# ygjwd12345/UCD

Measured on AMD Instinct MI355X. Metric: images/sec (whole node) per UCD train step, VOC 15-5 step-1, 513^2 bs=24, higher is better.
Workload: dtype bf16

## Files before the change

### include/ucd_hip.h

```cpp
#ifndef UCD_HIP_H
#define UCD_HIP_H

#include <stddef.h>
#include <stdint.h>

#ifdef __cplusplus
extern "C" {
#endif

#define UCD_VERSION 100

typedef void* ucd_stream_t;
typedef void* ucd_comm_t;

enum ucd_dtype { UCD_F32 = 0, UCD_BF16 = 1 };
enum ucd_act { UCD_ACT_IDENTITY = 0, UCD_ACT_LEAKY_RELU = 1, UCD_ACT_ELU = 2  };
#define UCD_ACT_MASK 0xff
#define UCD_NORM_ABS_GAMMA 0x100
enum ucd_pixcon_precision { UCD_PIXCON_F32 = 0, UCD_PIXCON_F16 = 1, UCD_PIXCON_F16_SPLIT = 2 };
enum ucd_error {
  UCD_OK = 0,
  UCD_EINVAL = -1,
  UCD_EALIGN = -2,
  UCD_EWORKSPACE = -3,
// ... 345 lines not shown
enum ucd_conv_form {
  UCD_CONV_SINGLE = 0,
  UCD_CONV_DB = 1,
  UCD_CONV_LW128 = 2,
  UCD_CONV_LW256 = 3,
  UCD_CONV_LW64 = 4
};
#define UCD_CONV_FORM_NAMES {"single", "2x64", "lw/128", "lw/256", "lw/64"}
typedef struct ucd_conv1x1_plan_t {
  int form;
  int tile_rows, tile_cols;
  int tiles_m, tiles_n, grid, threads, lds_bytes;
  int param_off;
} ucd_conv1x1_plan_t;
int ucd_conv1x1_plan(const ucd_conv1x1_desc* desc, ucd_conv1x1_plan_t* plan);
int ucd_conv1x1_row_tiles(int M);
int ucd_conv1x1_stat_replicas(int M);
size_t ucd_conv1x1_stats_partial_bytes(int M, int C);
int ucd_conv1x1(const ucd_conv1x1_desc* desc, ucd_stream_t stream);

int ucd_conv3_tap_plan(int B, int H, int W, int dilation, int tile_rows, int* perm, int* masks, int* n_classes);
int ucd_conv3_tap_classes(int mode);
int ucd_conv3_tap_plans_resident(void);
int ucd_conv3_tap_stats(long long* launches, int* last_tile_rows, int* last_class_ordered);

int ucd_conv1x1_stats_finalize(const float* partial, int M, int C, const float* weight, float* running_mean,
                               float* running_var, float momentum, float eps, float* buf, float* pack, int flags,
                               ucd_stream_t stream);

int ucd_abn_reduce_partials(const float* partial, int tiles, int C, float* sums, float* sums_copy, const float* weight,
// ... 105 lines not shown
```

### ucd_amd/csrc/conv1x1.hip

```cpp
#include "common.h"
#include "abn_finalize.h"
#include "conv3_taps.h"
#include <algorithm>
#include <mutex>
#include <vector>

namespace ucd {
namespace {

typedef float f32x16 __attribute__((ext_vector_type(16)));
typedef __bf16 bf16x8 __attribute__((ext_vector_type(8)));
typedef __hip_bfloat16 bf16;

constexpr int kThreads = 256;
constexpr int kBM = 128;

constexpr int kBK = 64;
constexpr int kDbStages = 2;
constexpr int kLwStages = 3;

struct Args {
  const bf16* A; int lda;
  const bf16* W; int ldw;
  bf16* Y; int ldy;
  int M, N, K;
  const float *in_mean, *in_scale, *in_shift; int in_act; float in_slope;
  const float *out_mean, *out_scale, *out_shift, *out_invstd;
// ... 29 lines not shown


template <int OUT> constexpr int kEpilogueBarriers = 4 + (OUT >= 2 ? 2 : 0);
template <int OUT, int HALVES> constexpr int kEpilogueBarriersH = 2 * HALVES + (OUT >= 2 ? 2 : 0);

__device__ __forceinline__ void live_taps(int m0, int m1, int ohw, int oW, int iH, int dil, int& tap0, int& ntap) {
  tap0 = 0; ntap = 9;
  if (dil <= 1 || m1 - m0 >= ohw) return;
  const int first = m0 % ohw, last = (m1 - 1) % ohw;
  int ymin = first / oW, ymax = last / oW;
  if (first > last) { ymin = 0; ymax = iH - 1; }
  if (ymax < dil) { tap0 = 3; ntap -= 3; }
  if (ymin >= iH - dil) ntap -= 3;
}

template <int BN, bool PRO, int OUT, bool CONV3 = false, bool DB = false, bool RT = false>
__global__ __launch_bounds__(kThreads, DB ? 2 : ((PRO || OUT >= 3) && BN == 128 ? 3 : 4)) void conv1x1_kernel(Args p) {
  static_assert(!DB || !PRO, "the double-buffered form has no input transform");
  static_assert(!RT || (CONV3 && OUT == 0 && !PRO), "class-ordered rows: the plain 3x3 product");
  constexpr int kStage = (kBM + BN) * kBK * 2;
  constexpr int WN = BN / 2;
  constexpr int TN = WN / 32;
  extern __shared__ __attribute__((aligned(1024))) unsigned char smem[];
  unsigned char* As = smem;
  unsigned char* Bs = smem + kBM * kBK * 2;
  float* Ps = reinterpret_cast<float*>(smem + p.param_off);

  const int xcd = blockIdx.x & 7, j = blockIdx.x >> 3;
  const int tm = (j / p.tiles_n) * 8 + xcd, tn = j % p.tiles_n;
  if (tm >= p.tiles_m) return;
  const int m0 = tm * kBM, n0 = tn * BN;
  const int tid = threadIdx.x, lane = tid & 63, wave = __builtin_amdgcn_readfirstlane(tid >> 6);
  const int wm = wave >> 1, wn = wave & 1;

  f32x16 acc[2][TN];
#pragma unroll
  for (int a = 0; a < 2; ++a)
#pragma unroll
    for (int b = 0; b < TN; ++b)
#pragma unroll
      for (int r = 0; r < 16; ++r) acc[a][b][r] = 0.f;

  constexpr int RPC = 1024 / (kBK * 2), SPR = kBK / 8;
  constexpr int CA = kBM / RPC / 4, CB = BN / RPC / 4;
  const bf16* ga[CA];
  const bf16* gb[CB];
  int py[CA], px[CA], pimg[CA], pslot[CA];
#pragma unroll
  for (int i = 0; i < CA; ++i) {
    const int row = RPC * (wave * CA + i) + lane / SPR;
    const int slot = ((lane % SPR) ^ swz_fn(row)) << 3;
    ga[i] = p.A + (size_t)min(m0 + row, p.M - 1) * p.lda + slot;
    if (CONV3 || p.stride > 1) {
      const int m = m0 + row;
      const int mm = min(m, p.M - 1);
      const int pix = RT ? p.perm[mm] : mm;
// ... 12 lines not shown
    gb[i] = p.W + (size_t)(n0 + row) * p.ldw + (((lane % SPR) ^ swz_fn(row)) << 3);
  }
  const int ks = tid & 7, srow = tid >> 3;
  const bf16* arow[4];
#pragma unroll
  for (int i = 0; i < 4; ++i) arow[i] = p.A + (size_t)min(m0 + srow + 32 * i, p.M - 1) * p.lda + ks * 8;

  if (PRO) {
    for (int k = tid; k < p.K; k += kThreads) {
      Ps[k] = p.in_mean[k];
      Ps[p.K + k] = p.in_scale[k];
      Ps[2 * p.K + k] = p.in_shift ? p.in_shift[k] : 0.f;
    }
    __syncthreads();
  }
  const int fr = lane & 31, fh = lane >> 5;
  const int kpt = p.K / kBK;
  int tap0 = 0, ntap = 9;
  unsigned trem = 0;
  if constexpr (RT) { trem = (unsigned)p.masks[tm]; ntap = __builtin_popcount(trem); }
  else if (CONV3 && p.stride == 1) live_taps(m0, min(m0 + kBM, p.M), p.ohw, p.oW, p.iH, p.dil, tap0, ntap);
  const int nk = CONV3 ? ntap * kpt : kpt;
  int akt = -1, ctap = 0;
  auto tap_of = [&](int kt) {
    if constexpr (RT) {
      if (kt != akt) { ctap = __builtin_ctz(trem); trem &= trem - 1; akt = kt; }
      return ctap;
    } else {
      return tap0 + kt;
    }
  };
// ... 103 lines not shown
      } else {
#pragma unroll
        for (int i = 0; i < CA; ++i)
          __builtin_amdgcn_raw_ptr_buffer_load_lds(rsA1, (lptr_t)(As + (wave * CA + i) * 1024), 16, (int)a1off[i], k0 * 2, 0, 0);
      }
#pragma unroll
      for (int i = 0; i < CB; ++i)
        __builtin_amdgcn_raw_ptr_buffer_load_lds(rsW, (lptr_t)(Bs + (wave * CB + i) * 1024), 16, (int)boff[i], wk0 * 2, 0, 0);
    }
    if (!DB) {
      if (!PRO) asm volatile("s_waitcnt vmcnt(0)" ::: "memory");
      asm volatile("s_waitcnt lgkmcnt(0)" ::: "memory");
      __builtin_amdgcn_s_barrier();
    }
    if (DB) {
      bf16x8 af[2][2], bfr[2][TN];
      auto read_slice = [&](int set, int kk) {
#pragma unroll
        for (int a = 0; a < 2; ++a) af[set][a] = *reinterpret_cast<const bf16x8*>(Ac + swz(wm * 64 + a * 32 + fr, 2 * kk + fh));
#pragma unroll
        for (int b = 0; b < TN; ++b) bfr[set][b] = *reinterpret_cast<const bf16x8*>(Bc + swz(wn * WN + b * 32 + fr, 2 * kk + fh));
      };
      read_slice(0, 0);
#pragma unroll
      for (int kk = 0; kk < kBK / 16; ++kk) {
        if (kk + 1 < kBK / 16) read_slice((kk + 1) & 1, kk + 1);
        __builtin_amdgcn_sched_barrier(0);
#pragma unroll
        for (int a = 0; a < 2; ++a)
#pragma unroll
          for (int b = 0; b < TN; ++b)
            acc[a][b] = __builtin_amdgcn_mfma_f32_32x32x16_bf16(af[kk & 1][a], bfr[kk & 1][b], acc[a][b], 0, 0, 0);
        __builtin_amdgcn_sched_barrier(0);
      }
    } else {
#pragma unroll
      for (int kk = 0; kk < kBK / 16; ++kk) {
        bf16x8 af[2], bfr[TN];
#pragma unroll
        for (int a = 0; a < 2; ++a) af[a] = *reinterpret_cast<const bf16x8*>(Ac + swz(wm * 64 + a * 32 + fr, 2 * kk + fh));
#pragma unroll
        for (int b = 0; b < TN; ++b) bfr[b] = *reinterpret_cast<const bf16x8*>(Bc + swz(wn * WN + b * 32 + fr, 2 * kk + fh));
#pragma unroll
        for (int a = 0; a < 2; ++a)
#pragma unroll
          for (int b = 0; b < TN; ++b) acc[a][b] = __builtin_amdgcn_mfma_f32_32x32x16_bf16(af[a], bfr[b], acc[a][b], 0, 0, 0);
      }
    }
  }

#include "conv1x1_epilogue.inc"
}

template <int BM, int BN, int OUT, bool CONV3, bool RT = false>
__global__ __launch_bounds__(BM == 64 ? 384 : BM * 4, (BM + BN) * kBK * 2 * kLwStages > 80 * 1024 ? 1 : 2) void conv_lw_kernel(Args p) {
  static_assert(BM == 64 || BM == 128 || BM == 256, "64-, 128- or 256-row workgroup tiles");
  static_assert(BM != 64 || BN == 64, "the 64-row form runs its epilogue on 128 threads: 64-column tiles");
  static_assert(!RT || (CONV3 && OUT == 0), "class-ordered rows: the plain 3x3 product");
  constexpr int NC = BM / 32, NL = BM == 64 ? 4 : BM / 32;
  constexpr int kStage = (BM + BN) * kBK * 2;
  constexpr int WN = BN / 2, TN = WN / 32;
  extern __shared__ __attribute__((aligned(1024))) unsigned char smem[];
  unsigned char* As = smem;
  unsigned char* Bs = smem + BM * kBK * 2;
  const int xcd = blockIdx.x & 7, j = blockIdx.x >> 3;
  const int tmw = (j / p.tiles_n) * 8 + xcd, tn = j % p.tiles_n;
  if (tmw >= p.tiles_m) return;
  const int m0w = tmw * BM, n0 = tn * BN;
  const int tid = threadIdx.x, lane = tid & 63, wave = __builtin_amdgcn_readfirstlane(tid >> 6);
  const int kpt = p.K / kBK;
  int tap0 = 0, ntap = 9;
  unsigned trem = 0;
  if constexpr (RT) { trem = (unsigned)p.masks[tmw]; ntap = __builtin_popcount(trem); }
  else if (CONV3 && p.stride == 1) live_taps(m0w, min(m0w + BM, p.M), p.ohw, p.oW, p.iH, p.dil, tap0, ntap);
  const int nk = CONV3 ? ntap * kpt : kpt;

// ... 72 lines not shown
    int wst = kLwStages - 1;
    for (int kb = 0; kb < nk; ++kb) {
      const int r = min(kLwStages - 2, nk - 1 - kb);
      if (r == 1) asm volatile("s_waitcnt vmcnt(%0)" ::"n"(CA + CB) : "memory");
      else asm volatile("s_waitcnt vmcnt(0)" ::: "memory");
      __builtin_amdgcn_s_barrier();
      if (kb + kLwStages - 1 < nk) fill(kb + kLwStages - 1, wst);
      wst = wst + 1 == kLwStages ? 0 : wst + 1;
    }
#pragma unroll
    for (int b = 0; b < kEpilogueBarriersH<OUT, BM == 64 ? 1 : 2>; ++b) __syncthreads();
    return;
  }

  const int wmw = wave >> 1, wn = wave & 1;
  f32x16 acc[2][TN];
#pragma unroll
  for (int a = 0; a < 2; ++a)
#pragma unroll
    for (int b = 0; b < TN; ++b)
#pragma unroll
      for (int r = 0; r < 16; ++r) acc[a][b][r] = 0.f;
  const int fr = lane & 31, fh = lane >> 5;
  int rst = 0;
  for (int kb = 0; kb < nk; ++kb) {
    asm volatile("s_waitcnt lgkmcnt(0)" ::: "memory");
    __builtin_amdgcn_s_barrier();
    const unsigned char* Ac = As + rst * kStage;
    const unsigned char* Bc = Bs + rst * kStage;
    rst = rst + 1 == kLwStages ? 0 : rst + 1;
    bf16x8 af[2][2], bfr[2][TN];
    auto read_slice = [&](int set, int kk) {
#pragma unroll
      for (int a = 0; a < 2; ++a) af[set][a] = *reinterpret_cast<const bf16x8*>(Ac + swz(wmw * 64 + a * 32 + fr, 2 * kk + fh));
#pragma unroll
      for (int b = 0; b < TN; ++b) bfr[set][b] = *reinterpret_cast<const bf16x8*>(Bc + swz(wn * WN + b * 32 + fr, 2 * kk + fh));
    };
    read_slice(0, 0);
#pragma unroll
    for (int kk = 0; kk < kBK / 16; ++kk) {
      if (kk + 1 < kBK / 16) read_slice((kk + 1) & 1, kk + 1);
      __builtin_amdgcn_sched_barrier(0);
#pragma unroll
      for (int a = 0; a < 2; ++a)
#pragma unroll
        for (int b = 0; b < TN; ++b)
          acc[a][b] = __builtin_amdgcn_mfma_f32_32x32x16_bf16(af[kk & 1][a], bfr[kk & 1][b], acc[a][b], 0, 0, 0);
      __builtin_amdgcn_sched_barrier(0);
    }
  }
  if constexpr (BM == 64) {
    const int tm = tmw, m0 = m0w, wm = 0;
#define UCD_EPI_THREADS 128
#define UCD_EPI_HALVES 1
#include "conv1x1_epilogue.inc"
#undef UCD_EPI_THREADS
#undef UCD_EPI_HALVES
  } else {
    const int sub = wmw >> 1;
    const int tm = tmw * (BM / 128) + sub, m0 = m0w + sub * 128, wm = wmw & 1;
    constexpr size_t kOutBytes = ((size_t)64 * (BN + 4) * 4 + 1023) / 1024 * 1024;
    unsigned char* smem_all = smem;
    {
// ... 282 lines not shown
        if (co + j < Co) q[j] = tmp[j];
    }
  }
}

int pick_wgrad_chunks(int M, int N, int K) {
  const int tiles = (N / 128) * (K / 128);
  int chunks = (512 + tiles - 1) / tiles;
  const int max_chunks = (M + 255) / 256;
  if (chunks > max_chunks) chunks = max_chunks;
  if (chunks < 1) chunks = 1;
  return chunks;
}


struct Tuning { int pipe, bn64_below, lw64_below; };
const Tuning& tuning() {
  static const Tuning t = [] {
    const char *e = getenv("UCD_CONV_PIPE"), *bn = getenv("UCD_CONV_BN64_TILES"), *lw = getenv("UCD_CONV_LW64_TILES");
    const int pipe = !e || !*e || !strcmp(e, "auto") ? -1 : !strcmp(e, "2x64") ? UCD_CONV_DB : !strcmp(e, "lw64") ? UCD_CONV_LW128
                     : !strcmp(e, "lw256") ? UCD_CONV_LW256 : -2;
    return Tuning{pipe, bn ? atoi(bn) : 128, lw ? atoi(lw) : 128};
  }();
  return t;
}

constexpr struct { int rows, threads, stages; } kForms[] = {{128, 256, 1}, {128, 256, kDbStages}, {128, 512, kLwStages},
                                                            {256, 1024, kLwStages}, {64, 384, kLwStages}};

int plan_launch(const ucd_conv1x1_desc* d, ucd_conv1x1_plan_t* p, const char* fn) {
  const Tuning& t = tuning();
  UCD_REQUIRE(t.pipe != -2, UCD_EINVAL, "%s: UCD_CONV_PIPE=%s names no form (accepted: auto, 2x64, lw64, lw256)", fn,
              getenv("UCD_CONV_PIPE"));
  const bool conv3 = d->taps == 9, pro = d->in_scale != nullptr;
  const int out = d->out_mode;
  UCD_REQUIRE(d->M > 0 && d->N > 0 && d->K > 0 && (d->taps == 0 || d->taps == 1 || conv3) && out >= 0 && out <= 4, UCD_EINVAL,
              "%s: empty product, taps not 1 or 9, or unknown out_mode", fn);
// ... 20 lines not shown
                         (size_t)(kThreads / (BN / 8)) * 2 * BN * 4});
  p->param_off = 0;
  if (pro) {
    p->param_off = (int)align_up(lds, 16);
    lds = p->param_off + (size_t)3 * d->K * sizeof(float);
  }
  UCD_REQUIRE(form != UCD_CONV_SINGLE || lds <= 64 * 1024, UCD_EUNSUPPORTED, "%s: K = %d is too wide for the fused input transform", fn,
              d->K);
  p->form = form; p->tile_rows = rows; p->tile_cols = BN;
  p->tiles_m = ceil_div(d->M, rows); p->tiles_n = tiles_n;
  p->grid = ceil_div(p->tiles_m, 8) * 8 * tiles_n;
  p->threads = kForms[form].threads; p->lds_bytes = (int)lds;
  return 0;
}

template <int BN, int OUT, bool CONV3, bool RT = false, bool PRO = false>
int launch_form(const ucd_conv1x1_plan_t& p, hipStream_t s, const Args& a, const char* fn) {
  const int lds = p.lds_bytes;
  if (p.form == UCD_CONV_SINGLE) {
    conv1x1_kernel<BN, PRO, OUT, CONV3, false, RT><<<p.grid, p.threads, lds, s>>>(a);
    return 0;
  }
  if constexpr (!PRO) {
    switch (p.form) {
      case UCD_CONV_DB:
        conv1x1_kernel<BN, false, OUT, CONV3, true, RT><<<p.grid, p.threads, lds, s>>>(a);
        return 0;
      case UCD_CONV_LW128:
        UCD_TRY_LDS((conv_lw_kernel<128, BN, OUT, CONV3, RT>), lds);
        conv_lw_kernel<128, BN, OUT, CONV3, RT><<<p.grid, p.threads, lds, s>>>(a);
        return 0;
      case UCD_CONV_LW256:
        if constexpr (OUT <= 2 && BN == 128) {
          UCD_TRY_LDS((conv_lw_kernel<256, BN, OUT, CONV3, RT>), lds);
          conv_lw_kernel<256, BN, OUT, CONV3, RT><<<p.grid, p.threads, lds, s>>>(a);
          return 0;
        }
        break;
      case UCD_CONV_LW64:
        if constexpr (BN == 64) {
          conv_lw_kernel<64, BN, OUT, CONV3, RT><<<p.grid, p.threads, lds, s>>>(a);
          return 0;
        }
        break;
    }
  }
  static const char* const names[] = UCD_CONV_FORM_NAMES;
  set_error("%s: no %s kernel for %d-column tiles and out_mode %d", fn, names[p.form], BN, OUT);
  return UCD_EINVAL;
}

template <int BN>
int launch_plan(const ucd_conv1x1_plan_t& p, int out_mode, bool conv3, bool pro, hipStream_t s, const Args& a, const char* fn) {
  UCD_REQUIRE(!(conv3 && out_mode == 4), UCD_EINVAL, "%s: out_mode 4 belongs to the 1x1 products", fn);
  UCD_REQUIRE(!(pro && (conv3 || out_mode == 4)), UCD_EINVAL, "%s: no input transform on a 3x3 product or with out_mode 4", fn);
  if (conv3) switch (out_mode) {
    case 0: return a.perm ? launch_form<BN, 0, true, true>(p, s, a, fn) : launch_form<BN, 0, true>(p, s, a, fn);
    case 1: return launch_form<BN, 1, true>(p, s, a, fn);
    case 2: return launch_form<BN, 2, true>(p, s, a, fn);
    default: return launch_form<BN, 3, true>(p, s, a, fn);
  }
  if (pro) switch (out_mode) {
    case 0: return launch_form<BN, 0, false, false, true>(p, s, a, fn);
    case 1: return launch_form<BN, 1, false, false, true>(p, s, a, fn);
    case 2: return launch_form<BN, 2, false, false, true>(p, s, a, fn);
    default: return launch_form<BN, 3, false, false, true>(p, s, a, fn);
  }
  switch (out_mode) {
    case 0: return launch_form<BN, 0, false>(p, s, a, fn);
    case 1: return launch_form<BN, 1, false>(p, s, a, fn);
    case 2: return launch_form<BN, 2, false>(p, s, a, fn);
    case 3: return launch_form<BN, 3, false>(p, s, a, fn);
    default: return launch_form<BN, 4, false>(p, s, a, fn);
  }
}

int g_tap_classes = -1;
std::mutex g_tap_mutex;
int tap_classes_mode() {
  std::lock_guard<std::mutex> lock(g_tap_mutex);
  if (g_tap_classes < 0) {
    const char* e = getenv("UCD_CONV3_TAP_CLASSES");
    g_tap_classes = e && !strcmp(e, "0") ? 0 : e && !strcmp(e, "2") ? 2 : 1;
  }
  return g_tap_classes;
}

struct TapPlan { int dev, B, H, W, d, rows; int* perm; int* masks; int max_on, max_off; };
// ... 125 lines not shown
  if (conv3 && stride == 1 && d->dilation > 1 && d->out_mode == 0) {
    const int mode = tap_classes_mode(), rows = plan.tile_rows;
    const TapPlan* tp = mode ? tap_plan_get(d->M / (d->H * d->W), d->H, d->W, d->dilation, rows, s) : nullptr;
    if (tp && mode == 1 && rows == 64 && tp->max_on >= tp->max_off) {
      int dev = 0, cus = 0;
      if (hipGetDevice(&dev) == hipSuccess && hipDeviceGetAttribute(&cus, hipDeviceAttributeMultiprocessorCount, dev) == hipSuccess &&
          (long long)plan.tiles_m * plan.tiles_n <= cus)
        tp = nullptr;
    }
    if (tp) { a.perm = tp->perm; a.masks = tp->masks; }
    std::lock_guard<std::mutex> lock(g_tap_mutex);
    g_tap_launches += tp != nullptr;
    g_tap_last_rows = rows; g_tap_last_rt = tp != nullptr;
  }
  const bool pro = d->in_scale != nullptr;
  if (int rc = plan.tile_cols == 128 ? launch_plan<128>(plan, d->out_mode, conv3, pro, s, a, fn)
                                     : launch_plan<64>(plan, d->out_mode, conv3, pro, s, a, fn))
    return rc;
  return check_launch(fn);
}

int ucd_conv1x1_plan(const ucd_conv1x1_desc* d, ucd_conv1x1_plan_t* plan) {
  static const char* fn = "ucd_conv1x1_plan";
  UCD_REQUIRE(d && plan, UCD_EINVAL, "%s: NULL argument", fn);
  return plan_launch(d, plan, fn);
}

int ucd_conv3_tap_classes(int mode) {
  const int cur = tap_classes_mode();
  if (mode < 0) return cur;
  std::lock_guard<std::mutex> lock(g_tap_mutex);
  g_tap_classes = mode >= 2 ? 2 : mode;
  return g_tap_classes;
}

int ucd_conv3_tap_stats(long long* launches, int* last_tile_rows, int* last_class_ordered) {
  std::lock_guard<std::mutex> lock(g_tap_mutex);
  if (launches) *launches = g_tap_launches;
  if (last_tile_rows) *last_tile_rows = g_tap_last_rows;
  if (last_class_ordered) *last_class_ordered = g_tap_last_rt;
// ... 102 lines not shown
```

### ucd_amd/csrc/conv1x1_epilogue.inc

```
#ifndef UCD_EPI_ACTIVE
#define UCD_EPI_ACTIVE true
#define UCD_EPI_ACTIVE_DEFAULTED
#endif
#ifndef UCD_EPI_TILE_OK
#define UCD_EPI_TILE_OK true
#define UCD_EPI_TILE_OK_DEFAULTED
#endif
#ifndef UCD_EPI_ROW
#define UCD_EPI_ROW(r) (r)
#endif
#ifndef UCD_EPI_THREADS
#define UCD_EPI_THREADS kThreads
#define UCD_EPI_HALVES 2
#define UCD_EPI_THREADS_DEFAULTED
#endif
  constexpr int CP = BN + 4;
  float* Cs = reinterpret_cast<float*>(smem);
  constexpr int CPR = BN / 8;
  constexpr int RPT = 64 * CPR / (UCD_EPI_THREADS);
  constexpr int RSTEP = (UCD_EPI_THREADS) / CPR;
  const int c8 = tid % CPR, r0 = tid / CPR;
  const int ncol = n0 + c8 * 8;
  Pack8 em, es, eb, ei;
  if (OUT == 3) {
    em = load_f8(p.out_mean + ncol);
    es = load_f8(p.out_scale + ncol);
    eb = load_f8(p.out_shift + ncol);
    ei = load_f8(p.out_invstd + ncol);
  }
  float am[OUT == 1 ? TN : 1], as_[OUT == 1 ? TN : 1], ab[OUT == 1 ? TN : 1];
  if (OUT == 1) {
#pragma unroll
    for (int b = 0; b < TN; ++b) {
      const int col = n0 + wn * WN + b * 32 + (lane & 31);
      am[b] = p.out_mean[col];
      as_[b] = p.out_scale[col];
      ab[b] = p.out_shift[col];
    }
  }
  if (OUT == 4) {
    em = load_f8(p.out_mean + ncol);
    ei = load_f8(p.out_invstd + ncol);
  }
  Pack8 kshift, s1, s2;
#pragma unroll
  for (int j = 0; j < 4; ++j) { kshift.p[j] = f32x2{0.f, 0.f}; s1.p[j] = f32x2{0.f, 0.f}; s2.p[j] = f32x2{0.f, 0.f}; }
  const bool has_side = ((OUT == 0 || OUT == 4) && p.accumulate) || (OUT == 1 && p.R != nullptr) || OUT == 3;
  const bf16* sp = (OUT == 0 || OUT == 4) ? p.Y : p.R;
  const int lds_ = (OUT == 0 || OUT == 4) ? p.ldy : p.ldr;
// ... 4 lines not shown
#pragma unroll
      for (int i = 0; i < RPT; ++i)
        side[i] = *reinterpret_cast<const uint4*>(sp + (size_t)UCD_EPI_ROW(min(m0 + half * 64 + r0 + RSTEP * i, p.M - 1)) * lds_ + ncol);
    }
    if (OUT == 4) {
#pragma unroll
      for (int i = 0; i < RPT; ++i) {
        const size_t row = (size_t)min(m0 + half * 64 + r0 + RSTEP * i, p.M - 1);
        side_y[i] = *reinterpret_cast<const uint4*>(p.R + row * p.ldr + ncol);
        side_z[i] = *reinterpret_cast<const uint4*>(p.Z + row * p.ldz + ncol);
      }
    }
    __syncthreads();
    if (wm == half) {
#pragma unroll
      for (int a = 0; a < 2; ++a)
#pragma unroll
        for (int b = 0; b < TN; ++b)
#pragma unroll
          for (int r = 0; r < 16; ++r) {
            const int row = a * 32 + (r & 3) + 8 * (r >> 2) + 4 * (lane >> 5);
            Cs[row * CP + wn * WN + b * 32 + (lane & 31)] =
                OUT == 1 ? (acc[a][b][r] - am[OUT == 1 ? b : 0]) * as_[OUT == 1 ? b : 0] + ab[OUT == 1 ? b : 0] : acc[a][b][r];
          }
    }
    __syncthreads();
    if (OUT == 2 && half == 0 && p.stat_acc) {
      kshift = load_f8(p.stat_shift + ncol);
    } else if (OUT == 2 && half == 0) {
      const float4 k0 = *reinterpret_cast<const float4*>(Cs + c8 * 8), k1 = *reinterpret_cast<const float4*>(Cs + c8 * 8 + 4);
      Pack8 kf;
      kf.p[0] = f32x2{k0.x, k0.y}; kf.p[1] = f32x2{k0.z, k0.w}; kf.p[2] = f32x2{k1.x, k1.y}; kf.p[3] = f32x2{k1.z, k1.w};
      kshift = unpack8(pack8(kf));
    }
#pragma unroll
    for (int i = 0; i < RPT; ++i) {
      const int row = r0 + RSTEP * i;
// ... 96 lines not shown
        dst[(1 + which) * p.N] = t;
      } else {
        p.partial[(size_t)tm * 2 * p.N + which * p.N + n0 + col] = t;
      }
    }
    if (OUT == 2 && p.stat_acc) {
      if (tm == 0 && r0 == 0 && UCD_EPI_TILE_OK) {
#pragma unroll
        for (int j = 0; j < 4; ++j) *reinterpret_cast<f32x2*>(p.partial + ncol + 2 * j) = kshift.p[j];
      }
    } else if (OUT == 2 && r0 == 0 && UCD_EPI_TILE_OK) {
#pragma unroll
      for (int j = 0; j < 4; ++j) *reinterpret_cast<f32x2*>(p.partial + (size_t)tm * 3 * p.N + ncol + 2 * j) = kshift.p[j];
    }
  }
#ifdef UCD_EPI_ACTIVE_DEFAULTED
#undef UCD_EPI_ACTIVE
#undef UCD_EPI_ACTIVE_DEFAULTED
#endif
#ifdef UCD_EPI_TILE_OK_DEFAULTED
#undef UCD_EPI_TILE_OK
#undef UCD_EPI_TILE_OK_DEFAULTED
#endif
#ifdef UCD_EPI_THREADS_DEFAULTED
#undef UCD_EPI_THREADS
#undef UCD_EPI_HALVES
#undef UCD_EPI_THREADS_DEFAULTED
#endif
```

### ucd_amd/hip.py

```python
from __future__ import annotations

import ctypes as C
import os

import torch

_HERE = os.path.dirname(os.path.abspath(__file__))
LIB_PATH = os.path.join(_HERE, "libucd_hip.so")

F32, BF16 = 0, 1
ACT_IDENTITY, ACT_LEAKY_RELU, ACT_ELU = 0, 1, 2
ACT_CODES = {"identity": ACT_IDENTITY, "leaky_relu": ACT_LEAKY_RELU, "elu": ACT_ELU}
ACT_MASK = 0xFF
NORM_ABS_GAMMA = 0x100
PIX_TILE = 128
PIXCON_LD = 256
PIXCON_F32, PIXCON_F16, PIXCON_F16_SPLIT = 0, 1, 2
KD_UNBIASED, KD_PLAIN = 0, 1
EINVAL, EALIGN, EWORKSPACE = -1, -2, -3
EUNSUPPORTED = -4
SEG_FORMS = {1: "pk<16,8>", 2: "pk<20,4>", 3: "pk<12,12>", 4: "reg<24,16>", 5: "reg<24,24>", 6: "wide/fixed", 7: "wide/f32"}
PIXCON_PATHS = {1: "f32", 2: "f32/wide", 3: "f16/planned", 4: "f16/split"}
CONV_FORMS = ("single", "2x64", "lw/128", "lw/256", "lw/64")
WGRAD_FORMS = ("tile", "strided", "row3")
# ... 97 lines not shown
    "ucd_pod_plan": (_i, [_i, _i, _i, _p, _i, _i, _i, _p, _p, _p]),
    "ucd_pod_forward": (_i, [_p, _i, _p, _i, _i, _i, _i, _i, _i, _f, _p, _i, _f, _p, _p, _p, _z, _p]),
    "ucd_pod_backward": (_i, [_p, _i, _i, _i, _i, _i, _i, _f, _p, _i, _p, _p, _p, _i, _p]),
    "ucd_pod_logits_plan": (_i, [_i, _i, _i, _i, _p, _i, _i, _i, _p, _p, _p]),
    "ucd_pod_logits_forward": (_i, [_p, _i, _p, _i, _i, _i, _i, _i, _i, _i, _p, _i, _i, _f, _p, _p, _p, _z, _p]),
    "ucd_pod_logits_backward": (_i, [_p, _i, _i, _i, _i, _i, _i, _i, _p, _i, _p, _p, _p, _i, _p]),
    "ucd_proto_plan": (_i, [_q, _i, _i, _i, _p, _p, _p, _p]),
    "ucd_proto_classify": (_i, [_p, _i, _i, _i, _i, _i, _i, _i, _i, _p, _i, _p, _p]),
    "ucd_proto_forward": (_i, [_p, _i, _i, _p, _q, _i, _i, _i, _p, _p, _p, _p, _f, _f, _f, _p, _p, _p, _p, _p, _z, _p]),
    "ucd_proto_backward": (_i, [_p, _i, _i, _p, _q, _i, _i, _p, _p, _p, _i, _p]),
    "ucd_proto_update": (_i, [_p, _p, _p, _p, _i, _i, _p]),
    "ucd_conv1x1_row_tiles": (_i, [_i]),
    "ucd_conv1x1_stats_partial_bytes": (_z, [_i, _i]),
    "ucd_conv1x1": (_i, [C.POINTER(Conv1x1Desc), _p]),
    "ucd_conv1x1_plan": (_i, [C.POINTER(Conv1x1Desc), C.POINTER(Conv1x1Plan)]),
    "ucd_conv1x1_stats_finalize": (_i, [_p, _i, _i, _p, _p, _p, _f, _f, _p, _p, _i, _p]),
    "ucd_conv3_tap_plan": (_i, [_i, _i, _i, _i, _i, _p, _p, _p]),
    "ucd_conv3_tap_classes": (_i, [_i]),
    "ucd_conv3_tap_plans_resident": (_i, []),
    "ucd_conv3_tap_stats": (_i, [_p, _p, _p]),
    "ucd_abn_reduce_partials": (_i, [_p, _i, _i, _p, _p, _p, _i, _p]),
    "ucd_conv1x1_wgrad_workspace_bytes": (_z, [_i, _i, _i]),
    "ucd_conv1x1_wgrad": (_i, [_p, _i, _p, _i, _i, _i, _i, _p, _p, _p, _i, _f, _p, _p, _z, _p]),
    "ucd_abn_sync_finalize": (_i, [_p, _i, _i, _i, _p, _p, _p, _f, _f, _p, _i, _p]),
    "ucd_stem_pooled_size": (_i, [_i]),
    "ucd_stem_pool_workspace_bytes": (_z, [_i]),
    "ucd_stem_apply_pool": (_i, [_p, _i, _i, _i, _i, _p, _p, _p, _i, _f, _p, _p, _p]),
    "ucd_stem_pool_backward": (_i, [_p, _p, _p, _i, _i, _i, _i, _p, _p, _p, _p, _p, _p, _f, _i, _f, _p, _p, _z, _i, _p]),
    "ucd_conv_wgrad_workspace_bytes": (_z, [_i, _i, _i, _i]),
    "ucd_stem_conv7x7": (_i, [_p, C.c_longlong, C.c_longlong, C.c_longlong, C.c_longlong, _i, _i, _i, _p, _p, _p]),
# ... 557 lines not shown
def _conv1x1_plan(d):
    p = Conv1x1Plan()
    _check(load().ucd_conv1x1_plan(C.byref(d), C.byref(p)), "ucd_conv1x1_plan")
    out = {n: getattr(p, n) for n, _ in Conv1x1Plan._fields_}
    out["form"] = CONV_FORMS[p.form]
    return out


def conv1x1_plan(M, N, K, taps=1, out_mode=0, stride=1, in_transform=False, stat_acc=False):
    d = Conv1x1Desc()
    d.M, d.N, d.K, d.taps, d.out_mode, d.stride = int(M), int(N), int(K), int(taps), int(out_mode), int(stride)
    d.in_scale, d.stat_acc = (16 if in_transform else None), (16 if stat_acc else None)
    return _conv1x1_plan(d)


def conv1x1(a, w, y, in_norm=None, out_mode=0, out_norm=None, residual=None, partial=None, accumulate=False, conv3=None,
            side2=None, strided=None, stat_acc=None, stat_shift=None, stat_acc2=None, stat_rep=1):
    lib = load()
    d = Conv1x1Desc()
    M, K = y.shape[0], a.shape[1]
    N = w.shape[0]
    d.a, d.lda, d.w, d.ldw, d.y, d.ldy = a.data_ptr(), a.stride(0), w.data_ptr(), w.stride(0), y.data_ptr(), y.stride(0)
    d.M, d.N, d.K = M, N, K
    if conv3 is not None:
        d.taps, d.H, d.W, d.dilation = 9, int(conv3[0]), int(conv3[1]), int(conv3[2])
        if len(conv3) > 3:
            d.stride = int(conv3[3])
    elif strided is not None:
        d.H, d.W, d.stride = int(strided[0]), int(strided[1]), int(strided[2])
    if in_norm is not None:
# ... 277 lines not shown
```

### ucd_amd/switches.py

```python
from __future__ import annotations

import os

DEFAULTS = {
    "UCD_FUSED_CONV1X1": "1",
    "UCD_BWD_LINK": "1",
    "UCD_BLOCK_LINK": "1",
    "UCD_PROJ_ALIAS": "1",
    "UCD_DGRAD_VIA_FWD": "1",
    "UCD_OWN_STRIDED": "1",
    "UCD_OWN_WGRAD": "1",
    "UCD_F32_OWN_CONV": "0",
    "UCD_OWN_HEADS": "1",
    "UCD_OWN_STEM": "1",
    "UCD_WGRAD3": "1",
    "UCD_CONV_PIPE": "auto",
    "UCD_CONV_BN64_TILES": "128",
    "UCD_CONV_LW64_TILES": "128",
    "UCD_WGRAD_DEFER": "1",
    "UCD_WGRAD_STREAM": "1",
    "UCD_CONV3_TAP_CLASSES": "1",
    "UCD_STAT_ATOMIC": "1",
    "UCD_SEG_PK": "1",
    "UCD_SEG_KD_EX": "1",
    "UCD_FUSED_LDE": "1",
    "UCD_FUSED_POD": "1",
    "UCD_FUSED_PSEUDO": "1",
    "UCD_FUSED_FOCAL": "1",
    "UCD_FUSED_PROTO": "1",
    "UCD_VAL_DEVICE": "1",
    "UCD_STEM_EVAL_FUSED": "1",
# ... 42 lines not shown
```

Measured before the change: 849.0.

## Add 16x16x32 MFMA variant for dilated 3x3 conv kernels with auto selection

Templates the conv GEMM kernels on the MFMA shape so they can use 16x16x32 bf16 instructions instead of 32x32x16. Adds a pipelined slice loop for the smaller shape and remaps the epilogue's accumulator rows and columns to match. A heuristic picks the 16-wide shape for dilated 3x3 products with large K and mid-sized grids, which is meant to help the ASPP-like layers. The trade is more LDS fragment reads and more instructions per tile in exchange for different issue and latency behaviour, plus more template instantiations.

```diff
diff --git a/include/ucd_hip.h b/include/ucd_hip.h
--- a/include/ucd_hip.h
+++ b/include/ucd_hip.h
@@ -383,6 +383,7 @@
   int param_off;
 } ucd_conv1x1_plan_t;
 int ucd_conv1x1_plan(const ucd_conv1x1_desc* desc, ucd_conv1x1_plan_t* plan);
+int ucd_conv1x1_mfma_shape(int M, int N, int K, int taps, int stride, int dilation);
 int ucd_conv1x1_row_tiles(int M);
 int ucd_conv1x1_stat_replicas(int M);
 size_t ucd_conv1x1_stats_partial_bytes(int M, int C);
diff --git a/ucd_amd/csrc/conv1x1.hip b/ucd_amd/csrc/conv1x1.hip
--- a/ucd_amd/csrc/conv1x1.hip
+++ b/ucd_amd/csrc/conv1x1.hip
@@ -11,6 +11,36 @@
 typedef float f32x16 __attribute__((ext_vector_type(16)));
 typedef __bf16 bf16x8 __attribute__((ext_vector_type(8)));
 typedef __hip_bfloat16 bf16;
+typedef float f32x4 __attribute__((ext_vector_type(4)));
+
+template <int MS> struct Mfma;
+template <> struct Mfma<32> { typedef f32x16 acc_t; static constexpr int kRegs = 16; };
+template <> struct Mfma<16> { typedef f32x4 acc_t; static constexpr int kRegs = 4; };
+#define UCD_MFMA(MS, acc, a, b)                                                            \
+  do {                                                                                     \
+    if constexpr ((MS) == 32) (acc) = __builtin_amdgcn_mfma_f32_32x32x16_bf16((a), (b), (acc), 0, 0, 0); \
+    else (acc) = __builtin_amdgcn_mfma_f32_16x16x32_bf16((a), (b), (acc), 0, 0, 0);        \
+  } while (0)
+
+#define UCD_SLICES_16(WM)                                                                                                       \
+  bf16x8 af[FA], bfr[2][FB];                                                                                                    \
+  _Pragma("unroll") for (int a = 0; a < FA; ++a)                                                                                \
+    af[a] = *reinterpret_cast<const bf16x8*>(Ac + swz((WM) * 64 + a * MS + fr, fh));                                            \
+  _Pragma("unroll") for (int b = 0; b < FB; ++b)                                                                                \
+    bfr[0][b] = *reinterpret_cast<const bf16x8*>(Bc + swz(wn * WN + b * MS + fr, fh));                                          \
+  _Pragma("unroll") for (int kk = 0; kk < KS; ++kk) {                                                                           \
+    if (kk + 1 < KS) {                                                                                                          \
+      _Pragma("unroll") for (int b = 0; b < FB; ++b)                                                                            \
+        bfr[(kk + 1) & 1][b] = *reinterpret_cast<const bf16x8*>(Bc + swz(wn * WN + b * MS + fr, SPS * (kk + 1) + fh));          \
+    }                                                                                                                           \
+    __builtin_amdgcn_sched_barrier(0);                                                                                          \
+    _Pragma("unroll") for (int a = 0; a < FA; ++a) {                                                                            \
+      _Pragma("unroll") for (int b = 0; b < FB; ++b) UCD_MFMA(MS, acc[a][b], af[a], bfr[kk & 1][b]);                            \
+      __builtin_amdgcn_sched_barrier(0);                                                                                        \
+      if (kk + 1 < KS) af[a] = *reinterpret_cast<const bf16x8*>(Ac + swz((WM) * 64 + a * MS + fr, SPS * (kk + 1) + fh));        \
+      __builtin_amdgcn_sched_barrier(0);                                                                                        \
+    }                                                                                                                           \
+  }
 
 constexpr int kThreads = 256;
 constexpr int kBM = 128;
@@ -70,13 +100,15 @@
   if (ymin >= iH - dil) ntap -= 3;
 }
 
-template <int BN, bool PRO, int OUT, bool CONV3 = false, bool DB = false, bool RT = false>
+template <int BN, bool PRO, int OUT, bool CONV3 = false, bool DB = false, bool RT = false, int MS = 32>
 __global__ __launch_bounds__(kThreads, DB ? 2 : ((PRO || OUT >= 3) && BN == 128 ? 3 : 4)) void conv1x1_kernel(Args p) {
   static_assert(!DB || !PRO, "the double-buffered form has no input transform");
   static_assert(!RT || (CONV3 && OUT == 0 && !PRO), "class-ordered rows: the plain 3x3 product");
+  static_assert(MS == 32 || (MS == 16 && !PRO), "MFMA shape: 32x32x16, or 16x16x32 in the forms without an input transform");
   constexpr int kStage = (kBM + BN) * kBK * 2;
   constexpr int WN = BN / 2;
-  constexpr int TN = WN / 32;
+  constexpr int FA = 64 / MS, FB = WN / MS;
+  constexpr int KS = MS / 8, SPS = 64 / MS;
   extern __shared__ __attribute__((aligned(1024))) unsigned char smem[];
   unsigned char* As = smem;
   unsigned char* Bs = smem + kBM * kBK * 2;
@@ -89,13 +121,13 @@
   const int tid = threadIdx.x, lane = tid & 63, wave = __builtin_amdgcn_readfirstlane(tid >> 6);
   const int wm = wave >> 1, wn = wave & 1;
 
-  f32x16 acc[2][TN];
-#pragma unroll
-  for (int a = 0; a < 2; ++a)
-#pragma unroll
-    for (int b = 0; b < TN; ++b)
-#pragma unroll
-      for (int r = 0; r < 16; ++r) acc[a][b][r] = 0.f;
+  typename Mfma<MS>::acc_t acc[FA][FB];
+#pragma unroll
+  for (int a = 0; a < FA; ++a)
+#pragma unroll
+    for (int b = 0; b < FB; ++b)
+#pragma unroll
+      for (int r = 0; r < Mfma<MS>::kRegs; ++r) acc[a][b][r] = 0.f;
 
   constexpr int RPC = 1024 / (kBK * 2), SPR = kBK / 8;
   constexpr int CA = kBM / RPC / 4, CB = BN / RPC / 4;
@@ -138,7 +170,7 @@
     }
     __syncthreads();
   }
-  const int fr = lane & 31, fh = lane >> 5;
+  const int fr = lane & (MS - 1), fh = lane >> (MS == 32 ? 5 : 4);
   const int kpt = p.K / kBK;
   int tap0 = 0, ntap = 9;
   unsigned trem = 0;
@@ -272,37 +304,40 @@
       __builtin_amdgcn_s_barrier();
     }
     if (DB) {
-      bf16x8 af[2][2], bfr[2][TN];
+      if constexpr (MS == 32) {
+      bf16x8 af[2][FA], bfr[2][FB];
       auto read_slice = [&](int set, int kk) {
 #pragma unroll
-        for (int a = 0; a < 2; ++a) af[set][a] = *reinterpret_cast<const bf16x8*>(Ac + swz(wm * 64 + a * 32 + fr, 2 * kk + fh));
-#pragma unroll
-        for (int b = 0; b < TN; ++b) bfr[set][b] = *reinterpret_cast<const bf16x8*>(Bc + swz(wn * WN + b * 32 + fr, 2 * kk + fh));
+        for (int a = 0; a < FA; ++a) af[set][a] = *reinterpret_cast<const bf16x8*>(Ac + swz(wm * 64 + a * MS + fr, SPS * kk + fh));
+#pragma unroll
+        for (int b = 0; b < FB; ++b) bfr[set][b] = *reinterpret_cast<const bf16x8*>(Bc + swz(wn * WN + b * MS + fr, SPS * kk + fh));
       };
       read_slice(0, 0);
 #pragma unroll
-      for (int kk = 0; kk < kBK / 16; ++kk) {
-        if (kk + 1 < kBK / 16) read_slice((kk + 1) & 1, kk + 1);
+      for (int kk = 0; kk < KS; ++kk) {
+        if (kk + 1 < KS) read_slice((kk + 1) & 1, kk + 1);
         __builtin_amdgcn_sched_barrier(0);
 #pragma unroll
-        for (int a = 0; a < 2; ++a)
-#pragma unroll
-          for (int b = 0; b < TN; ++b)
-            acc[a][b] = __builtin_amdgcn_mfma_f32_32x32x16_bf16(af[kk & 1][a], bfr[kk & 1][b], acc[a][b], 0, 0, 0);
+        for (int a = 0; a < FA; ++a)
+#pragma unroll
+          for (int b = 0; b < FB; ++b) UCD_MFMA(MS, acc[a][b], af[kk & 1][a], bfr[kk & 1][b]);
         __builtin_amdgcn_sched_barrier(0);
       }
+      } else {
+        UCD_SLICES_16(wm)
+      }
     } else {
 #pragma unroll
-      for (int kk = 0; kk < kBK / 16; ++kk) {
-        bf16x8 af[2], bfr[TN];
-#pragma unroll
-        for (int a = 0; a < 2; ++a) af[a] = *reinterpret_cast<const bf16x8*>(Ac + swz(wm * 64 + a * 32 + fr, 2 * kk + fh));
-#pragma unroll
-        for (int b = 0; b < TN; ++b) bfr[b] = *reinterpret_cast<const bf16x8*>(Bc + swz(wn * WN + b * 32 + fr, 2 * kk + fh));
-#pragma unroll
-        for (int a = 0; a < 2; ++a)
-#pragma unroll
-          for (int b = 0; b < TN; ++b) acc[a][b] = __builtin_amdgcn_mfma_f32_32x32x16_bf16(af[a], bfr[b], acc[a][b], 0, 0, 0);
+      for (int kk = 0; kk < KS; ++kk) {
+        bf16x8 af[FA], bfr[FB];
+#pragma unroll
+        for (int a = 0; a < FA; ++a) af[a] = *reinterpret_cast<const bf16x8*>(Ac + swz(wm * 64 + a * MS + fr, SPS * kk + fh));
+#pragma unroll
+        for (int b = 0; b < FB; ++b) bfr[b] = *reinterpret_cast<const bf16x8*>(Bc + swz(wn * WN + b * MS + fr, SPS * kk + fh));
+#pragma unroll
+        for (int a = 0; a < FA; ++a)
+#pragma unroll
+          for (int b = 0; b < FB; ++b) UCD_MFMA(MS, acc[a][b], af[a], bfr[b]);
       }
     }
   }
@@ -310,14 +345,15 @@
 #include "conv1x1_epilogue.inc"
 }
 
-template <int BM, int BN, int OUT, bool CONV3, bool RT = false>
+template <int BM, int BN, int OUT, bool CONV3, bool RT = false, int MS = 32>
 __global__ __launch_bounds__(BM == 64 ? 384 : BM * 4, (BM + BN) * kBK * 2 * kLwStages > 80 * 1024 ? 1 : 2) void conv_lw_kernel(Args p) {
   static_assert(BM == 64 || BM == 128 || BM == 256, "64-, 128- or 256-row workgroup tiles");
   static_assert(BM != 64 || BN == 64, "the 64-row form runs its epilogue on 128 threads: 64-column tiles");
   static_assert(!RT || (CONV3 && OUT == 0), "class-ordered rows: the plain 3x3 product");
   constexpr int NC = BM / 32, NL = BM == 64 ? 4 : BM / 32;
   constexpr int kStage = (BM + BN) * kBK * 2;
-  constexpr int WN = BN / 2, TN = WN / 32;
+  static_assert(MS == 32 || MS == 16, "MFMA shape: 32x32x16 or 16x16x32");
+  constexpr int WN = BN / 2, FA = 64 / MS, FB = WN / MS, KS = MS / 8, SPS = 64 / MS;
   extern __shared__ __attribute__((aligned(1024))) unsigned char smem[];
   unsigned char* As = smem;
   unsigned char* Bs = smem + BM * kBK * 2;
@@ -420,14 +456,14 @@
   }
 
   const int wmw = wave >> 1, wn = wave & 1;
-  f32x16 acc[2][TN];
-#pragma unroll
-  for (int a = 0; a < 2; ++a)
-#pragma unroll
-    for (int b = 0; b < TN; ++b)
-#pragma unroll
-      for (int r = 0; r < 16; ++r) acc[a][b][r] = 0.f;
-  const int fr = lane & 31, fh = lane >> 5;
+  typename Mfma<MS>::acc_t acc[FA][FB];
+#pragma unroll
+  for (int a = 0; a < FA; ++a)
+#pragma unroll
+    for (int b = 0; b < FB; ++b)
+#pragma unroll
+      for (int r = 0; r < Mfma<MS>::kRegs; ++r) acc[a][b][r] = 0.f;
+  const int fr = lane & (MS - 1), fh = lane >> (MS == 32 ? 5 : 4);
   int rst = 0;
   for (int kb = 0; kb < nk; ++kb) {
     asm volatile("s_waitcnt lgkmcnt(0)" ::: "memory");
@@ -435,24 +471,27 @@
     const unsigned char* Ac = As + rst * kStage;
     const unsigned char* Bc = Bs + rst * kStage;
     rst = rst + 1 == kLwStages ? 0 : rst + 1;
-    bf16x8 af[2][2], bfr[2][TN];
+    if constexpr (MS == 32) {
+    bf16x8 af[2][FA], bfr[2][FB];
     auto read_slice = [&](int set, int kk) {
 #pragma unroll
-      for (int a = 0; a < 2; ++a) af[set][a] = *reinterpret_cast<const bf16x8*>(Ac + swz(wmw * 64 + a * 32 + fr, 2 * kk + fh));
-#pragma unroll
-      for (int b = 0; b < TN; ++b) bfr[set][b] = *reinterpret_cast<const bf16x8*>(Bc + swz(wn * WN + b * 32 + fr, 2 * kk + fh));
+      for (int a = 0; a < FA; ++a) af[set][a] = *reinterpret_cast<const bf16x8*>(Ac + swz(wmw * 64 + a * MS + fr, SPS * kk + fh));
+#pragma unroll
+      for (int b = 0; b < FB; ++b) bfr[set][b] = *reinterpret_cast<const bf16x8*>(Bc + swz(wn * WN + b * MS + fr, SPS * kk + fh));
     };
     read_slice(0, 0);
 #pragma unroll
-    for (int kk = 0; kk < kBK / 16; ++kk) {
-      if (kk + 1 < kBK / 16) read_slice((kk + 1) & 1, kk + 1);
+    for (int kk = 0; kk < KS; ++kk) {
+      if (kk + 1 < KS) read_slice((kk + 1) & 1, kk + 1);
       __builtin_amdgcn_sched_barrier(0);
 #pragma unroll
-      for (int a = 0; a < 2; ++a)
-#pragma unroll
-        for (int b = 0; b < TN; ++b)
-          acc[a][b] = __builtin_amdgcn_mfma_f32_32x32x16_bf16(af[kk & 1][a], bfr[kk & 1][b], acc[a][b], 0, 0, 0);
+      for (int a = 0; a < FA; ++a)
+#pragma unroll
+        for (int b = 0; b < FB; ++b) UCD_MFMA(MS, acc[a][b], af[kk & 1][a], bfr[kk & 1][b]);
       __builtin_amdgcn_sched_barrier(0);
+    }
+    } else {
+      UCD_SLICES_16(wmw)
     }
   }
   if constexpr (BM == 64) {
@@ -765,13 +804,15 @@
 }
 
 
-struct Tuning { int pipe, bn64_below, lw64_below; };
+struct Tuning { int pipe, bn64_below, lw64_below, mfma; };
 const Tuning& tuning() {
   static const Tuning t = [] {
     const char *e = getenv("UCD_CONV_PIPE"), *bn = getenv("UCD_CONV_BN64_TILES"), *lw = getenv("UCD_CONV_LW64_TILES");
+    const char* ms = getenv("UCD_CONV_MFMA");
+    const int mfma = !ms || !*ms || !strcmp(ms, "auto") ? 0 : !strcmp(ms, "32") ? 32 : !strcmp(ms, "16") ? 16 : -2;
     const int pipe = !e || !*e || !strcmp(e, "auto") ? -1 : !strcmp(e, "2x64") ? UCD_CONV_DB : !strcmp(e, "lw64") ? UCD_CONV_LW128
                      : !strcmp(e, "lw256") ? UCD_CONV_LW256 : -2;
-    return Tuning{pipe, bn ? atoi(bn) : 128, lw ? atoi(lw) : 128};
+    return Tuning{pipe, bn ? atoi(bn) : 128, lw ? atoi(lw) : 128, mfma};
   }();
   return t;
 }
@@ -822,32 +863,42 @@
   return 0;
 }
 
-template <int BN, int OUT, bool CONV3, bool RT = false, bool PRO = false>
+int mfma_shape(int M, int N, int K, int taps, int stride, int dilation, const char* fn) {
+  const Tuning& t = tuning();
+  UCD_REQUIRE(t.mfma != -2, UCD_EINVAL, "%s: UCD_CONV_MFMA=%s names no MFMA shape (accepted: auto, 32, 16)", fn, getenv("UCD_CONV_MFMA"));
+  UCD_REQUIRE(M > 0 && N > 0 && K > 0 && (taps == 0 || taps == 1 || taps == 9), UCD_EINVAL, "%s: empty product or taps not 1 or 9", fn);
+  if (t.mfma) return t.mfma;
+  const long long wg128 = (long long)ceil_div(M, kBM) * (N / 128), wg256 = (long long)ceil_div(M, 256) * (N / 128);
+  if (taps == 9 && stride <= 1 && dilation > 1 && N % 128 == 0 && K >= 2048 && wg128 > 256 && wg128 <= 640 && wg256 <= 256) return 16;
+  return 32;
+}
+
+template <int BN, int OUT, bool CONV3, bool RT = false, bool PRO = false, int MS = 32>
 int launch_form(const ucd_conv1x1_plan_t& p, hipStream_t s, const Args& a, const char* fn) {
   const int lds = p.lds_bytes;
   if (p.form == UCD_CONV_SINGLE) {
-    conv1x1_kernel<BN, PRO, OUT, CONV3, false, RT><<<p.grid, p.threads, lds, s>>>(a);
+    conv1x1_kernel<BN, PRO, OUT, CONV3, false, RT, MS><<<p.grid, p.threads, lds, s>>>(a);
     return 0;
   }
   if constexpr (!PRO) {
     switch (p.form) {
       case UCD_CONV_DB:
-        conv1x1_kernel<BN, false, OUT, CONV3, true, RT><<<p.grid, p.threads, lds, s>>>(a);
+        conv1x1_kernel<BN, false, OUT, CONV3, true, RT, MS><<<p.grid, p.threads, lds, s>>>(a);
         return 0;
       case UCD_CONV_LW128:
-        UCD_TRY_LDS((conv_lw_kernel<128, BN, OUT, CONV3, RT>), lds);
-        conv_lw_kernel<128, BN, OUT, CONV3, RT><<<p.grid, p.threads, lds, s>>>(a);
+        UCD_TRY_LDS((conv_lw_kernel<128, BN, OUT, CONV3, RT, MS>), lds);
+        conv_lw_kernel<128, BN, OUT, CONV3, RT, MS><<<p.grid, p.threads, lds, s>>>(a);
         return 0;
       case UCD_CONV_LW256:
         if constexpr (OUT <= 2 && BN == 128) {
-          UCD_TRY_LDS((conv_lw_kernel<256, BN, OUT, CONV3, RT>), lds);
-          conv_lw_kernel<256, BN, OUT, CONV3, RT><<<p.grid, p.threads, lds, s>>>(a);
+          UCD_TRY_LDS((conv_lw_kernel<256, BN, OUT, CONV3, RT, MS>), lds);
+          conv_lw_kernel<256, BN, OUT, CONV3, RT, MS><<<p.grid, p.threads, lds, s>>>(a);
           return 0;
         }
         break;
       case UCD_CONV_LW64:
         if constexpr (BN == 64) {
-          conv_lw_kernel<64, BN, OUT, CONV3, RT><<<p.grid, p.threads, lds, s>>>(a);
+          conv_lw_kernel<64, BN, OUT, CONV3, RT, MS><<<p.grid, p.threads, lds, s>>>(a);
           return 0;
         }
         break;
@@ -858,15 +909,16 @@
   return UCD_EINVAL;
 }
 
-template <int BN>
+template <int BN, int MS>
 int launch_plan(const ucd_conv1x1_plan_t& p, int out_mode, bool conv3, bool pro, hipStream_t s, const Args& a, const char* fn) {
   UCD_REQUIRE(!(conv3 && out_mode == 4), UCD_EINVAL, "%s: out_mode 4 belongs to the 1x1 products", fn);
   UCD_REQUIRE(!(pro && (conv3 || out_mode == 4)), UCD_EINVAL, "%s: no input transform on a 3x3 product or with out_mode 4", fn);
   if (conv3) switch (out_mode) {
-    case 0: return a.perm ? launch_form<BN, 0, true, true>(p, s, a, fn) : launch_form<BN, 0, true>(p, s, a, fn);
-    case 1: return launch_form<BN, 1, true>(p, s, a, fn);
-    case 2: return launch_form<BN, 2, true>(p, s, a, fn);
-    default: return launch_form<BN, 3, true>(p, s, a, fn);
+    case 0: return a.perm ? launch_form<BN, 0, true, true, false, MS>(p, s, a, fn)
+                          : launch_form<BN, 0, true, false, false, MS>(p, s, a, fn);
+    case 1: return launch_form<BN, 1, true, false, false, MS>(p, s, a, fn);
+    case 2: return launch_form<BN, 2, true, false, false, MS>(p, s, a, fn);
+    default: return launch_form<BN, 3, true, false, false, MS>(p, s, a, fn);
   }
   if (pro) switch (out_mode) {
     case 0: return launch_form<BN, 0, false, false, true>(p, s, a, fn);
@@ -875,11 +927,11 @@
     default: return launch_form<BN, 3, false, false, true>(p, s, a, fn);
   }
   switch (out_mode) {
-    case 0: return launch_form<BN, 0, false>(p, s, a, fn);
-    case 1: return launch_form<BN, 1, false>(p, s, a, fn);
-    case 2: return launch_form<BN, 2, false>(p, s, a, fn);
-    case 3: return launch_form<BN, 3, false>(p, s, a, fn);
-    default: return launch_form<BN, 4, false>(p, s, a, fn);
+    case 0: return launch_form<BN, 0, false, false, false, MS>(p, s, a, fn);
+    case 1: return launch_form<BN, 1, false, false, false, MS>(p, s, a, fn);
+    case 2: return launch_form<BN, 2, false, false, false, MS>(p, s, a, fn);
+    case 3: return launch_form<BN, 3, false, false, false, MS>(p, s, a, fn);
+    default: return launch_form<BN, 4, false, false, false, MS>(p, s, a, fn);
   }
 }
 
@@ -1035,8 +1087,12 @@
     g_tap_last_rows = rows; g_tap_last_rt = tp != nullptr;
   }
   const bool pro = d->in_scale != nullptr;
-  if (int rc = plan.tile_cols == 128 ? launch_plan<128>(plan, d->out_mode, conv3, pro, s, a, fn)
-                                     : launch_plan<64>(plan, d->out_mode, conv3, pro, s, a, fn))
+  const int ms = mfma_shape(d->M, d->N, d->K, d->taps, stride, conv3 ? d->dilation : 1, fn);
+  if (ms < 0) return ms;
+  if (int rc = ms == 16 && !pro ? (plan.tile_cols == 128 ? launch_plan<128, 16>(plan, d->out_mode, conv3, pro, s, a, fn)
+                                                         : launch_plan<64, 16>(plan, d->out_mode, conv3, pro, s, a, fn))
+                                : (plan.tile_cols == 128 ? launch_plan<128, 32>(plan, d->out_mode, conv3, pro, s, a, fn)
+                                                         : launch_plan<64, 32>(plan, d->out_mode, conv3, pro, s, a, fn)))
     return rc;
   return check_launch(fn);
 }
@@ -1045,6 +1101,10 @@
   static const char* fn = "ucd_conv1x1_plan";
   UCD_REQUIRE(d && plan, UCD_EINVAL, "%s: NULL argument", fn);
   return plan_launch(d, plan, fn);
+}
+
+int ucd_conv1x1_mfma_shape(int M, int N, int K, int taps, int stride, int dilation) {
+  return mfma_shape(M, N, K, taps, stride > 1 ? stride : 1, dilation > 1 ? dilation : 1, "ucd_conv1x1_mfma_shape");
 }
 
 int ucd_conv3_tap_classes(int mode) {
diff --git a/ucd_amd/csrc/conv1x1_epilogue.inc b/ucd_amd/csrc/conv1x1_epilogue.inc
--- a/ucd_amd/csrc/conv1x1_epilogue.inc
+++ b/ucd_amd/csrc/conv1x1_epilogue.inc
@@ -9,6 +9,8 @@
 #ifndef UCD_EPI_ROW
 #define UCD_EPI_ROW(r) (r)
 #endif
+#define UCD_EPI_ACC_ROW(a, r) (MS == 32 ? (a) * 32 + ((r) & 3) + 8 * ((r) >> 2) + 4 * (lane >> 5) : (a) * 16 + 4 * (lane >> 4) + (r))
+#define UCD_EPI_ACC_COL(b) (wn * WN + (b) * MS + (lane & (MS - 1)))
 #ifndef UCD_EPI_THREADS
 #define UCD_EPI_THREADS kThreads
 #define UCD_EPI_HALVES 2
@@ -28,11 +30,11 @@
     eb = load_f8(p.out_shift + ncol);
     ei = load_f8(p.out_invstd + ncol);
   }
-  float am[OUT == 1 ? TN : 1], as_[OUT == 1 ? TN : 1], ab[OUT == 1 ? TN : 1];
+  float am[OUT == 1 ? FB : 1], as_[OUT == 1 ? FB : 1], ab[OUT == 1 ? FB : 1];
   if (OUT == 1) {
 #pragma unroll
-    for (int b = 0; b < TN; ++b) {
-      const int col = n0 + wn * WN + b * 32 + (lane & 31);
+    for (int b = 0; b < FB; ++b) {
+      const int col = n0 + UCD_EPI_ACC_COL(b);
       am[b] = p.out_mean[col];
       as_[b] = p.out_scale[col];
       ab[b] = p.out_shift[col];
@@ -67,13 +69,13 @@
     __syncthreads();
     if (wm == half) {
 #pragma unroll
-      for (int a = 0; a < 2; ++a)
-#pragma unroll
-        for (int b = 0; b < TN; ++b)
-#pragma unroll
-          for (int r = 0; r < 16; ++r) {
-            const int row = a * 32 + (r & 3) + 8 * (r >> 2) + 4 * (lane >> 5);
-            Cs[row * CP + wn * WN + b * 32 + (lane & 31)] =
+      for (int a = 0; a < FA; ++a)
+#pragma unroll
+        for (int b = 0; b < FB; ++b)
+#pragma unroll
+          for (int r = 0; r < Mfma<MS>::kRegs; ++r) {
+            const int row = UCD_EPI_ACC_ROW(a, r);
+            Cs[row * CP + UCD_EPI_ACC_COL(b)] =
                 OUT == 1 ? (acc[a][b][r] - am[OUT == 1 ? b : 0]) * as_[OUT == 1 ? b : 0] + ab[OUT == 1 ? b : 0] : acc[a][b][r];
           }
     }
@@ -200,6 +202,8 @@
       for (int j = 0; j < 4; ++j) *reinterpret_cast<f32x2*>(p.partial + (size_t)tm * 3 * p.N + ncol + 2 * j) = kshift.p[j];
     }
   }
+#undef UCD_EPI_ACC_ROW
+#undef UCD_EPI_ACC_COL
 #ifdef UCD_EPI_ACTIVE_DEFAULTED
 #undef UCD_EPI_ACTIVE
 #undef UCD_EPI_ACTIVE_DEFAULTED
diff --git a/ucd_amd/hip.py b/ucd_amd/hip.py
--- a/ucd_amd/hip.py
+++ b/ucd_amd/hip.py
@@ -135,6 +135,7 @@
     "ucd_conv1x1_stats_partial_bytes": (_z, [_i, _i]),
     "ucd_conv1x1": (_i, [C.POINTER(Conv1x1Desc), _p]),
     "ucd_conv1x1_plan": (_i, [C.POINTER(Conv1x1Desc), C.POINTER(Conv1x1Plan)]),
+    "ucd_conv1x1_mfma_shape": (_i, [_i] * 6),
     "ucd_conv1x1_stats_finalize": (_i, [_p, _i, _i, _p, _p, _p, _f, _f, _p, _p, _i, _p]),
     "ucd_conv3_tap_plan": (_i, [_i, _i, _i, _i, _i, _p, _p, _p]),
     "ucd_conv3_tap_classes": (_i, [_i]),
@@ -722,6 +723,13 @@
     return _conv1x1_plan(d)
 
 
+def conv1x1_mfma_shape(M, N, K, taps=1, stride=1, dilation=1):
+    ms = load().ucd_conv1x1_mfma_shape(int(M), int(N), int(K), int(taps), int(stride), int(dilation))
+    if ms < 0:
+        _check(ms, "ucd_conv1x1_mfma_shape")
+    return ms
+
+
 def conv1x1(a, w, y, in_norm=None, out_mode=0, out_norm=None, residual=None, partial=None, accumulate=False, conv3=None,
             side2=None, strided=None, stat_acc=None, stat_shift=None, stat_acc2=None, stat_rep=1):
     lib = load()
diff --git a/ucd_amd/switches.py b/ucd_amd/switches.py
--- a/ucd_amd/switches.py
+++ b/ucd_amd/switches.py
@@ -15,6 +15,7 @@
     "UCD_OWN_STEM": "1",
     "UCD_WGRAD3": "1",
     "UCD_CONV_PIPE": "auto",
+    "UCD_CONV_MFMA": "auto",
     "UCD_CONV_BN64_TILES": "128",
     "UCD_CONV_LW64_TILES": "128",
     "UCD_WGRAD_DEFER": "1",
```

New measurement: 847.4. Within noise of the previous version (-0.2%).
